# strukturag/libde265

Hardware: NVIDIA H100
Metric: decoded frames/sec at 4K Main profile, bit-exact YUV; MC kernel HBM GB/s (higher is better)
Workload: dtype u8

## Files before the change

libde265_b200/csrc/kernels_recon.cuh:

```cuda
#pragma once
#include "dev_common.cuh"
#include "kernels_residual.cuh"

#define RC_WARPS 8
#define RC_THREADS (RC_WARPS * 32)
#define RC_GSTRIDE 34
#define RC_TILE_STRIDE 40
#define RC_BLK (33 * RC_TILE_STRIDE + 8)
#define RC_FULL 0xffffffffu
#define RC_TRACE_WORDS 8

struct ReconArgs {
  const b200_tu* tus;
  const uint32_t* list;
  int n_list;
  int poll_ns;
  int region;
  int n_listw, n_list8;
  const uint32_t* task_start;
  int n_task;
  const b200_coeff* coeffs;
  const uint8_t* scaling;
  unsigned int* ticket;
  unsigned long long* trace;
  uint8_t* pend[3];
  int pend_w[3];
  const uint32_t* mark_list;
  int n_mark;
  unsigned int* err;
  unsigned int* err_host;
  unsigned long long spin_limit_ns;
};

struct ResidualSmem {
  int16_t coef[RC_WARPS][32 * RC_GSTRIDE];
  int16_t g[RC_WARPS][32 * RC_GSTRIDE];
  ResTables tb;
};

template <typename P>
struct IntraSmem {
  P blk[RC_WARPS][RC_BLK];
  int16_t coef[RC_WARPS][32 * RC_GSTRIDE];
  int16_t g[RC_WARPS][32 * RC_GSTRIDE];
  res_t res[RC_WARPS][32 * 32];
  P border[RC_WARPS][2][4 * 32 + 4];
  b200_tu tu_s[RC_WARPS][16];
  ResTables tb;
};

template <typename P, bool TO_RES>
__device__ void tu_residual(const b200_tu& tu, const b200_coeff* co, const uint8_t* __restrict__ scaling, P* dst, int dstride, res_t* res,
                            int bd, int16_t* coefT, int16_t* g, const ResTables& tb, int lane)
{
  const int log2 = tu.log2_size, nT = 1 << log2, n = tu.n_coeff;
  const int flags = tu.flags;
  const bool special = flags & (B200_TU_BYPASS | B200_TU_TSKIP);
  const Dequant dq = dequant_setup(tu, scaling, bd);
  int max_row = 0, max_col = 0;
  if (special) {
    max_row = max_col = nT - 1;
  } else {
    for (int i = lane; i < n; i += 32) {
      const int pos = co[i].pos;
      max_row = max(max_row, pos >> log2);
      max_col = max(max_col, pos & (nT - 1));
    }
    max_row = __reduce_max_sync(RC_FULL, max_row) & (nT - 1);
    max_col = __reduce_max_sync(RC_FULL, max_col) & (nT - 1);
  }
  const int nq = (max_row >> 2) + 1;
  uint32_t* cw = reinterpret_cast<uint32_t*>(coefT);
  uint32_t* gw = reinterpret_cast<uint32_t*>(g);
  constexpr int CW = RC_GSTRIDE / 2;
  for (int o = lane; o < (max_col + 1) * 2 * nq; o += 32) cw[(o / (2 * nq)) * CW + o % (2 * nq)] = 0;
  __syncwarp();
  for (int i = lane; i < n; i += 32) {
    const b200_coeff c = co[i];
    const int v = dequant_level(dq, c);
    const int pos = (dq.rotate ? (nT * nT - 1 - c.pos) : c.pos) & (nT * nT - 1);
    coefT[(pos & (nT - 1)) * RC_GSTRIDE + (pos >> log2)] = (int16_t)v;
  }
  __syncwarp();

  auto emit4 = [&](int x, int y, const int (&r)[4]) {
    if (TO_RES) res_store4(res + x + (y << log2), r[0], r[1], r[2], r[3]);
    else add_row<P, 4>(dst + x + (size_t)y * dstride, r, bd);
  };

  if (special) {
    const bool ts = !(flags & B200_TU_BYPASS);
    const int bd_shift = 20 - bd, ts_shift = 5 + log2, rnd = 1 << (bd_shift - 1);
    auto value = [&](int x, int y) {
      int c = coefT[x * RC_GSTRIDE + y];
      if (ts) c = ((int)((unsigned)c << ts_shift) + rnd) >> bd_shift;
      return c;
    };
    if (flags & (B200_TU_RDPCM_H | B200_TU_RDPCM_V)) {
      const bool vert = flags & B200_TU_RDPCM_V;
      if (lane < nT) {
        int sum = 0;
        for (int k = 0; k < nT; k++) {
          const int x = vert ? lane : k, y = vert ? k : lane;
          sum += value(x, y);
          if (TO_RES) res[x + (y << log2)] = (res_t)clip16(sum);
          else dst[x + (size_t)y * dstride] = (P)clip_bd((int)dst[x + (size_t)y * dstride] + sum, bd);
        }
      }
    } else {
      for (int o = lane; o < nT * nT / 4; o += 32) {
        const int x = (o & (nT / 4 - 1)) * 4, y = o >> (log2 - 2);
        const int r[4] = {value(x, y), value(x + 1, y), value(x + 2, y), value(x + 3, y)};
        emit4(x, y, r);
      }
    }
    __syncwarp();
    return;
  }

  const uint32_t* mt = (nT == 32) ? &tb.m32[0][0] : &tb.m16[0][0];
  const int post_shift = 20 - bd, rnd2 = 1 << (post_shift - 1);
  for (int o = lane; o < (max_col + 1) << (log2 - 2); o += 32) {
    const int ib = o & (nT / 4 - 1), c = o >> (log2 - 2);
    int acc[4] = {64, 64, 64, 64};
    const uint32_t* cp = cw + c * CW;
    for (int jq = 0; jq < nq; jq++) {
      const uint32_t c0 = cp[2 * jq], c1 = cp[2 * jq + 1];
      const uint4 m = *reinterpret_cast<const uint4*>(mt + jq * nT + 4 * ib);
      acc[0] = dp2a_hi(c1, m.x, dp2a_lo(c0, m.x, acc[0]));
      acc[1] = dp2a_hi(c1, m.y, dp2a_lo(c0, m.y, acc[1]));
      acc[2] = dp2a_hi(c1, m.z, dp2a_lo(c0, m.z, acc[2]));
      acc[3] = dp2a_hi(c1, m.w, dp2a_lo(c0, m.w, acc[3]));
    }
#pragma unroll
    for (int r = 0; r < 4; r++) g[(4 * ib + r) * RC_GSTRIDE + c] = (int16_t)clip16(acc[r] >> 7);
  }
  if ((max_col & 3) != 3) {
    const int c0 = max_col + 1, nc = 3 - (max_col & 3);
    for (int o = lane; o < nT * nc; o += 32) g[(o / nc) * RC_GSTRIDE + c0 + o % nc] = 0;
  }
  __syncwarp();
  const int nq2 = (max_col >> 2) + 1;
  for (int o = lane; o < nT << (log2 - 2); o += 32) {
    const int ib = o & (nT / 4 - 1), y = o >> (log2 - 2);
    int acc[4] = {rnd2, rnd2, rnd2, rnd2};
    const uint32_t* gp = gw + y * CW;
    for (int jq = 0; jq < nq2; jq++) {
      const uint32_t g0 = gp[2 * jq], g1 = gp[2 * jq + 1];
      const uint4 m = *reinterpret_cast<const uint4*>(mt + jq * nT + 4 * ib);
      acc[0] = dp2a_hi(g1, m.x, dp2a_lo(g0, m.x, acc[0]));
      acc[1] = dp2a_hi(g1, m.y, dp2a_lo(g0, m.y, acc[1]));
      acc[2] = dp2a_hi(g1, m.z, dp2a_lo(g0, m.z, acc[2]));
      acc[3] = dp2a_hi(g1, m.w, dp2a_lo(g0, m.w, acc[3]));
    }
    const int r[4] = {acc[0] >> post_shift, acc[1] >> post_shift, acc[2] >> post_shift, acc[3] >> post_shift};
    emit4(4 * ib, y, r);
  }
  __syncwarp();
}

__constant__ int8_t k_intra_angle[35] = {0,   0,   32,  26,  21,  17, 13, 9,  5,  2,  0,  -2, -5, -9, -13, -17, -21, -26,
                                         -32, -26, -21, -17, -13, -9, -5, -2, 0,  2,  5,  9,  13, 17, 21,  26,  32};
__constant__ int16_t k_inv_angle[15] = {-4096, -1638, -910, -630, -482, -390, -315, -256, -315, -390, -482, -630, -910, -1638, -4096};

template <typename P>
__device__ __forceinline__ void tu_intra_small(const b200_tu& tu, P* dst, int ts, int bd, bool filter_plane, const res_t* res, int lane)
{
  const int log2 = tu.log2_size, nT = 1 << log2, mode = tu.intra_mode, cidx = tu.cidx;
  const uint64_t avail = tu.avail;
  const int total = 4 * nT + 1;
  int v = 0, ve = 0;
  bool av = false, av_e = false;
  {
    const int i = lane - 2 * nT;
    if (lane < total) {
      if (i < 0) { const int r = -i - 1; av = (avail >> (r >> 2)) & 1; if (av) v = dst[-1 + r * ts]; }
      else if (i == 0) { av = (avail >> B200_AVAIL_CORNER_BIT) & 1; if (av) v = dst[-1 - ts]; }
      else { const int c = i - 1; av = (avail >> (B200_AVAIL_TOP_BIT0 + (c >> 2))) & 1; if (av) v = dst[c - ts]; }
    }
    if (nT == 8) {
      av_e = (avail >> (B200_AVAIL_TOP_BIT0 + 3)) & 1;
      if (av_e) ve = dst[15 - ts];
    }
  }
  {
    const unsigned m = __ballot_sync(RC_FULL, av);
    if (m == 0 && !av_e) {
      v = ve = 1 << (bd - 1);
    } else {
      const int first_lane = m ? __ffs(m) - 1 : 0;
      const int fv = __shfl_sync(RC_FULL, v, first_lane);
      const int first = m ? fv : ve;
      const unsigned below = m & ((2u << lane) - 1u);
      const int sv = __shfl_sync(RC_FULL, v, below ? 31 - __clz(below) : 0);
      v = below ? sv : first;
      const int last = __shfl_sync(RC_FULL, v, 31);
      if (!av_e) ve = last;
    }
  }
  if (filter_plane && nT == 8 && mode != 1) {
    const int d = min(abs(mode - 26), abs(mode - 10));
    if (d > 7) {
      const int vm = __shfl_up_sync(RC_FULL, v, 1);
      int vp = __shfl_down_sync(RC_FULL, v, 1);
      if (lane == 31) vp = ve;
      if (lane != 0) v = (vp + 2 * v + vm + 2) >> 2;
    }
  }
  auto B = [&](int i) -> int {
    const int s = i + 2 * nT;
    const int r = __shfl_sync(RC_FULL, v, s & 31);
    return (s == 32) ? ve : r;
  };
  const int npass = (nT == 4) ? 1 : 2;
  if (mode == 0) {
    const int tr = B(1 + nT), bl = B(-1 - nT);
    for (int p = 0; p < npass; p++) {
      const int o = lane + 32 * p, x = o & (nT - 1), y = (o >> log2) & (nT - 1);
      const int l = B(-1 - y), t = B(1 + x);
      int px = ((nT - 1 - x) * l + (x + 1) * tr + (nT - 1 - y) * t + (y + 1) * bl + nT) >> (log2 + 1);
      if (o < nT * nT) {
        if (res) px = clip_bd(px + res[o], bd);
        dst[x + y * ts] = (P)px;
      }
    }
  } else if (mode == 1) {
    const int i = lane - 2 * nT;
    const bool in = (i >= 1 && i <= nT) || (i <= -1 && i >= -nT);
    const int dc = (__reduce_add_sync(RC_FULL, in ? v : 0) + nT) >> (log2 + 1);
    const bool edge = (cidx == 0);
    const int b1 = B(1), bm1 = B(-1);
    for (int p = 0; p < npass; p++) {
      const int o = lane + 32 * p, x = o & (nT - 1), y = (o >> log2) & (nT - 1);
      const int t = B(x + 1), l = B(-y - 1);
      int px = dc;
      if (edge) {
        if (x == 0 && y == 0) px = (bm1 + 2 * dc + b1 + 2) >> 2;
        else if (y == 0) px = (t + 3 * dc + 2) >> 2;
        else if (x == 0) px = (l + 3 * dc + 2) >> 2;
      }
      if (o < nT * nT) {
        if (res) px = clip_bd(px + res[o], bd);
        dst[x + y * ts] = (P)px;
      }
    }
  } else {
    const int angle = k_intra_angle[mode];
    const bool vert = mode >= 18;
    const int sgn = vert ? 1 : -1;
    const int inv = (angle < 0) ? (int)k_inv_angle[mode - 11] : 0;
    const bool bfilt = (cidx == 0 && !(tu.flags & B200_TU_NO_BOUNDARY_FILTER) && (mode == 26 || mode == 10));
    const int b0 = B(0), b1 = B(1), bm1 = B(-1);
    auto R = [&](int k) -> int { return B(k >= 0 ? sgn * k : -sgn * ((k * inv + 128) >> 8)); };
    for (int p = 0; p < npass; p++) {
      const int o = lane + 32 * p, x = o & (nT - 1), y = (o >> log2) & (nT - 1);
      const int a = vert ? y : x, b = vert ? x : y;
      const int idx = ((a + 1) * angle) >> 5, fact = ((a + 1) * angle) & 31;
      const int r1 = R(b + idx + 1), r2 = R(b + idx + 2);
      const int l = B(-1 - y), t = B(1 + x);
      int px = fact ? ((32 - fact) * r1 + fact * r2 + 16) >> 5 : r1;
      if (bfilt) {
        if (mode == 26 && x == 0) px = clip_bd(b1 + ((l - b0) >> 1), bd);
        if (mode == 10 && y == 0) px = clip_bd(bm1 + ((t - b0) >> 1), bd);
      }
      if (o < nT * nT) {
        if (res) px = clip_bd(px + res[o], bd);
        dst[x + y * ts] = (P)px;
      }
    }
  }
  __syncwarp();
}

__device__ __forceinline__ bool intra_border_clamps(const b200_tu& tu, int& lo, int& hi)
{
  const int q = 1 << (tu.log2_size - 2);
  const uint64_t g = (1ull << q) - 1, av = tu.avail;
  if ((av & g) != g || !((av >> B200_AVAIL_CORNER_BIT) & 1) || ((av >> B200_AVAIL_TOP_BIT0) & g) != g) return false;
  const unsigned bl = (unsigned)((av >> q) & g), tr = (unsigned)((av >> (B200_AVAIL_TOP_BIT0 + q)) & g);
  if ((bl & (bl + 1)) || (tr & (tr + 1))) return false;
  lo = -4 * (q + __popc(bl));
  hi = 4 * (q + __popc(tr));
  return true;
}

struct TuDesc {
  uint32_t a, b;
  __device__ __forceinline__ int toff() const { return a & 1023; }
  __device__ __forceinline__ int mode() const { return (a >> 10) & 63; }
  __device__ __forceinline__ bool big() const { return (a >> 16) & 1; }
  __device__ __forceinline__ bool fast() const { return (a >> 17) & 1; }
  __device__ __forceinline__ bool smooth() const { return (a >> 18) & 1; }
  __device__ __forceinline__ bool bfilt() const { return (a >> 19) & 1; }
  __device__ __forceinline__ bool cbf() const { return (a >> 21) & 1; }
  __device__ __forceinline__ int rbase() const { return a >> 22; }
  __device__ __forceinline__ int plan_class() const { return (int)b; }
};

#define INTRA_PLAN_CLASSES (2 * 35 * 4 * 4 * 8)
__device__ uint32_t g_intra_plan[INTRA_PLAN_CLASSES][64];

inline void intra_plan_words(int cls, int lane, uint32_t (&w)[2])
{
  static const int8_t angle_of[35] = {0,   0,   32,  26,  21,  17, 13, 9,  5,  2,  0,  -2, -5, -9, -13, -17, -21, -26,
                                      -32, -26, -21, -17, -13, -9, -5, -2, 0,  2,  5,  9,  13, 17, 21,  26,  32};
  static const int16_t inv_of[15] = {-4096, -1638, -910, -630, -482, -390, -315, -256, -315, -390, -482, -630, -910, -1638, -4096};
  const bool smooth = cls & 1, bfilt = (cls >> 1) & 1, luma = (cls >> 2) & 1;
  const int hi2 = 4 * (((cls >> 3) & 3) + 1), lo2 = -4 * (((cls >> 5) & 3) + 1), mode = (cls >> 7) % 35, big = (cls >> 7) / 35;
  const int nT = big ? 8 : 4, log2 = big ? 3 : 2;
  auto O = [&](int i) -> uint32_t { i = std::min(std::max(i, lo2), hi2); return (uint32_t)(i < 0 ? -i * RC_TILE_STRIDE : i); };
  auto taps = [&](int i) -> uint32_t {
    if (smooth && i > -2 * nT && i < 2 * nT) return O(i - 1) | O(i) << 10 | O(i + 1) << 20;
    return O(i) * (1u | 1u << 10 | 1u << 20);
  };
  for (int p = 0; p < 2; p++) {
    const int o = lane + 32 * p, x = o & (nT - 1), y = (o >> log2) & (nT - 1);
    uint32_t v = 0;
    if (mode == 0) {
      if (p == 0 && lane <= 2 * nT + 2) v = taps(lane - nT - 1);
    } else if (mode == 1) {
      if (luma) {
        if (x == 0 && y == 0) v = O(-1) | O(1) << 10 | 2u << 20;
        else if (y == 0) v = O(x + 1) | 1u << 20;
        else if (x == 0) v = O(-y - 1) | 1u << 20;
      }
      const int i = lane - nT;
      if (p == 0 && lane < 2 * nT) v |= O(i < 0 ? i : i + 1) << 22;
    } else {
      const int angle = angle_of[mode], inv = angle < 0 ? inv_of[mode - 11] : 0, sgn = mode >= 18 ? 1 : -1;
      const int a = mode >= 18 ? y : x, b = mode >= 18 ? x : y;
      const int idx = ((a + 1) * angle) >> 5, fact = ((a + 1) * angle) & 31;
      auto R = [&](int k) -> int { return k >= 0 ? sgn * k : -sgn * ((k * inv + 128) >> 8); };
      if (smooth) v = taps(R(b + idx + 1));
      else v = O(R(b + idx + 1)) | O(R(b + idx + 2)) << 10 | (uint32_t)fact << 20;
      if (bfilt && mode == 26 && x == 0) v = O(1) | O(-1 - y) << 10 | 1u << 31;
      if (bfilt && mode == 10 && y == 0) v = O(-1) | O(1 + x) << 10 | 1u << 31;
    }
    w[p] = v;
  }
}

__device__ __forceinline__ TuDesc tu_desc(const b200_tu& tu, int G, bool filter_plane, int rbase)
{
  const int nT = 1 << tu.log2_size, mode = tu.intra_mode;
  int lo2 = 0, hi2 = 0;
  const bool fast = intra_border_clamps(tu, lo2, hi2);
  const bool smooth = nT == 8 && filter_plane && mode != 1 && min(abs(mode - 26), abs(mode - 10)) > 7;
  const bool bfilt = tu.cidx == 0 && !(tu.flags & B200_TU_NO_BOUNDARY_FILTER) && (mode == 26 || mode == 10);
  TuDesc d;
  d.a = (uint32_t)((tu.y & (G - 1)) * RC_TILE_STRIDE + (tu.x & (G - 1))) | (uint32_t)mode << 10 | (uint32_t)(nT == 8) << 16 | (uint32_t)fast << 17 |
        (uint32_t)smooth << 18 | (uint32_t)bfilt << 19 | (uint32_t)(tu.cidx == 0) << 20 | (uint32_t)((tu.flags & B200_TU_CBF) != 0) << 21 |
        (uint32_t)rbase << 22;
  d.b = fast ? (uint32_t)(((((nT == 8) * 35 + mode) * 4 + (-lo2 / 4 - 1)) * 4 + (hi2 / 4 - 1)) * 8 + (smooth | bfilt << 1 | (tu.cidx == 0) << 2)) : 0u;
  return d;
}

__device__ __forceinline__ TuDesc shfl_desc(const TuDesc& d, int src)
{
  return TuDesc{__shfl_sync(RC_FULL, d.a, src), __shfl_sync(RC_FULL, d.b, src)};
}

template <typename P, int LOG2>
__device__ __forceinline__ void tu_intra_fast(const TuDesc& d, P* dst, int ts, int bd, const int (&r)[2], const uint32_t (&w)[2], int lane)
{
  constexpr int nT = 1 << LOG2;
  constexpr int NP = (nT == 4) ? 1 : 2;
  const P* org = dst - ts - 1;
  auto T = [&](uint32_t u) -> int { return (int)org[u & 1023]; };
  auto F = [&](uint32_t u) -> int { return (T(u) + 2 * T(u >> 10) + T(u >> 20) + 2) >> 2; };
  const int mode = d.mode();
  int px[NP];
  if (mode == 0) {
    const int f = F(w[0]);
    const int tr = __shfl_sync(RC_FULL, f, 2 * nT + 2), bl = __shfl_sync(RC_FULL, f, 0);
#pragma unroll
    for (int p = 0; p < NP; p++) {
      const int o = lane + 32 * p, x = o & (nT - 1), y = (o >> LOG2) & (nT - 1);
      const int l = __shfl_sync(RC_FULL, f, nT - y), t = __shfl_sync(RC_FULL, f, nT + 2 + x);
      px[p] = ((nT - 1 - x) * l + (x + 1) * tr + (nT - 1 - y) * t + (y + 1) * bl + nT) >> (LOG2 + 1);
    }
  } else if (mode == 1) {
    const int dc = (__reduce_add_sync(RC_FULL, lane < 2 * nT ? T(w[0] >> 22) : 0) + nT) >> (LOG2 + 1);
#pragma unroll
    for (int p = 0; p < NP; p++) {
      const int kind = (w[p] >> 20) & 3, a = T(w[p]), b = kind == 2 ? T(w[p] >> 10) : dc;
      px[p] = kind ? (a + b + 2 * dc + 2) >> 2 : dc;
    }
  } else if (nT == 8 && d.smooth()) {
#pragma unroll
    for (int p = 0; p < NP; p++) px[p] = F(w[p]);
  } else {
#pragma unroll
    for (int p = 0; p < NP; p++) {
      const int r1 = T(w[p]), r2 = T(w[p] >> 10), fact = (w[p] >> 20) & 31;
      px[p] = ((32 - fact) * r1 + fact * r2 + 16) >> 5;
      if (d.bfilt() && (w[p] >> 31)) px[p] = clip_bd(r1 + ((r2 - (int)org[0]) >> 1), bd);
    }
  }
#pragma unroll
  for (int p = 0; p < NP; p++) {
    const int o = lane + 32 * p, x = o & (nT - 1), y = (o >> LOG2) & (nT - 1);
    if (o < nT * nT) dst[x + y * ts] = (P)clip_bd(px[p] + r[p], bd);
  }
  __syncwarp();
}

template <typename P>
__device__ void tu_intra_large(const b200_tu& tu, const P* gsrc, int gstride, P* dst, int bd, int bd_luma, uint32_t pic_flags, bool filter_plane,
                               P* b0mem, P* b1mem, int lane)
{
  const int log2 = tu.log2_size, nT = 1 << log2, mode = tu.intra_mode, cidx = tu.cidx, dstride = nT;
  const uint64_t avail = tu.avail;
  P* b0 = b0mem + 2 * 32 + 2;
  P* b1 = b1mem + 2 * 32 + 2;
  const int total = 4 * nT + 1;
  {
    constexpr int MAXC = 5;
    int v[MAXC];
    bool av[MAXC];
#pragma unroll
    for (int c5 = 0; c5 < MAXC; c5++) {
      const int s = 32 * c5 + lane, i = s - 2 * nT;
      av[c5] = false;
      v[c5] = 0;
      if (s < total) {
        const P* addr;
        if (i < 0) { const int r = -i - 1; av[c5] = (avail >> (r >> 2)) & 1; addr = gsrc - 1 + r * gstride; }
        else if (i == 0) { av[c5] = (avail >> B200_AVAIL_CORNER_BIT) & 1; addr = gsrc - 1 - gstride; }
        else { const int c = i - 1; av[c5] = (avail >> (B200_AVAIL_TOP_BIT0 + (c >> 2))) & 1; addr = gsrc + c - gstride; }
        if (av[c5]) v[c5] = (int)__ldcg(addr);
      }
    }
    int first_val = 1 << (bd - 1);
    bool any = false;
#pragma unroll
    for (int c5 = 0; c5 < MAXC; c5++) {
      const unsigned m = __ballot_sync(0xffffffffu, av[c5]);
      if (!any && m) { first_val = __shfl_sync(0xffffffffu, v[c5], __ffs(m) - 1); any = true; }
    }
    if (!any) {
      for (int s = lane; s < total; s += 32) b0[s - 2 * nT] = (P)(1 << (bd - 1));
    } else {
      int carry = first_val;
#pragma unroll
      for (int c5 = 0; c5 < MAXC; c5++) {
        if (32 * c5 < total) {
          const int s = 32 * c5 + lane, i = s - 2 * nT;
          const unsigned m = __ballot_sync(0xffffffffu, av[c5]);
          const unsigned below = m & ((2u << lane) - 1u);
          const int src = below ? 31 - __clz(below) : 0;
          const int sv = __shfl_sync(0xffffffffu, v[c5], src);
          const int outv = below ? sv : carry;
          if (s < total) b0[i] = (P)outv;
          carry = __shfl_sync(0xffffffffu, outv, 31);
        }
      }
    }
  }
  __syncwarp();
  const P* bsrc = b0;
  if (filter_plane && mode != 1) {
    const int d = min(abs(mode - 26), abs(mode - 10));
    const bool filt = d > ((nT == 8) ? 7 : (nT == 16) ? 1 : 0);
    if (filt) {
      const bool strong = (pic_flags & B200_PIC_STRONG_INTRA_SMOOTHING) && cidx == 0 && nT == 32 &&
                          abs((int)b0[0] + (int)b0[64] - 2 * (int)b0[32]) < (1 << (bd_luma - 5)) &&
                          abs((int)b0[0] + (int)b0[-64] - 2 * (int)b0[-32]) < (1 << (bd_luma - 5));
      for (int s = lane; s < total; s += 32) {
        const int i = s - 2 * nT;
        int v;
        if (i == -2 * nT || i == 2 * nT) v = b0[i];
        else if (strong) {
          if (i == 0) v = b0[0];
          else if (i < 0) v = (int)b0[0] + (((-i) * ((int)b0[-64] - (int)b0[0]) + 32) >> 6);
          else v = (int)b0[0] + ((i * ((int)b0[64] - (int)b0[0]) + 32) >> 6);
        } else v = ((int)b0[i + 1] + 2 * (int)b0[i] + (int)b0[i - 1] + 2) >> 2;
        b1[i] = (P)v;
      }
      __syncwarp();
      bsrc = b1;
    }
  }
  P* bfree = (bsrc == b0) ? b1 : b0;
  if (mode == 0) {
    for (int o = lane; o < nT * nT; o += 32) {
      const int x = o & (nT - 1), y = o >> log2;
      dst[x + y * dstride] = (P)(((nT - 1 - x) * (int)bsrc[-1 - y] + (x + 1) * (int)bsrc[1 + nT] + (nT - 1 - y) * (int)bsrc[1 + x] +
                                  (y + 1) * (int)bsrc[-1 - nT] + nT) >> (log2 + 1));
    }
  } else if (mode == 1) {
    int part = 0;
    for (int i = lane; i < nT; i += 32) part += (int)bsrc[i + 1] + (int)bsrc[-i - 1];
    const int dc = (__reduce_add_sync(RC_FULL, part) + nT) >> (log2 + 1);
    const bool edge = (cidx == 0 && nT < 32);
    for (int o = lane; o < nT * nT; o += 32) {
      const int x = o & (nT - 1), y = o >> log2;
      int v = dc;
      if (edge) {
        if (x == 0 && y == 0) v = ((int)bsrc[-1] + 2 * dc + (int)bsrc[1] + 2) >> 2;
        else if (y == 0) v = ((int)bsrc[x + 1] + 3 * dc + 2) >> 2;
        else if (x == 0) v = ((int)bsrc[-y - 1] + 3 * dc + 2) >> 2;
      }
      dst[x + y * dstride] = (P)v;
    }
  } else {
    const int angle = k_intra_angle[mode];
    const bool vert = mode >= 18;
    const int sgn = vert ? 1 : -1;
    P* ref = bfree;
    const int last = (nT * angle) >> 5;
    const int inv = (angle < 0) ? (int)k_inv_angle[mode - 11] : 0;
    const bool project = (angle < 0) && (last < -1);
    for (int s = lane; s <= 3 * nT; s += 32) {
      const int x = s - nT;
      const bool w = (x >= 0) ? (x <= nT || angle >= 0) : (project && x >= last);
      const int idx = (x >= 0) ? sgn * x : -sgn * ((x * inv + 128) >> 8);
      if (w) ref[x] = bsrc[idx];
    }
    __syncwarp();
    const bool bfilt = (cidx == 0 && nT < 32 && !(tu.flags & B200_TU_NO_BOUNDARY_FILTER) && (mode == 26 || mode == 10));
    for (int o = lane; o < nT * nT; o += 32) {
      const int x = o & (nT - 1), y = o >> log2;
      const int a = vert ? y : x, b = vert ? x : y;
      const int idx = ((a + 1) * angle) >> 5, fact = ((a + 1) * angle) & 31;
      int v = fact ? ((32 - fact) * (int)ref[b + idx + 1] + fact * (int)ref[b + idx + 2] + 16) >> 5 : (int)ref[b + idx + 1];
      if (bfilt) {
        if (mode == 26 && x == 0) v = clip_bd((int)bsrc[1] + (((int)bsrc[-1 - y] - (int)bsrc[0]) >> 1), bd);
        if (mode == 10 && y == 0) v = clip_bd((int)bsrc[-1] + (((int)bsrc[1 + x] - (int)bsrc[0]) >> 1), bd);
      }
      dst[x + y * dstride] = (P)v;
    }
  }
  __syncwarp();
}

template <typename P>
__device__ void tu_intra_large_clamped(const b200_tu& tu, int lo, int hi, P* gdst, int gstride, int bd, int bd_luma, uint32_t pic_flags,
                                       bool filter_plane, const res_t* res, P* bmem, int lane)
{
  const int log2 = tu.log2_size, nT = 1 << log2, mode = tu.intra_mode, cidx = tu.cidx;
  const int total = 4 * nT + 1;
  P* bs = bmem + 2 * 32 + 2;
  constexpr int MAXC = 5;
  int v[MAXC];
#pragma unroll
  for (int c5 = 0; c5 < MAXC; c5++) {
    const int s = 32 * c5 + lane, i = min(max(s - 2 * nT, lo), hi);
    v[c5] = 0;
    if (s < total) v[c5] = (int)__ldcg(i < 0 ? gdst - 1 + (-i - 1) * gstride : gdst + (i - 1) - gstride);
  }
  const bool filt = filter_plane && mode != 1 && min(abs(mode - 26), abs(mode - 10)) > ((nT == 16) ? 1 : 0);
  bool strong = false;
  int c0 = 0, bl = 0, tr = 0;
  if (filt && (pic_flags & B200_PIC_STRONG_INTRA_SMOOTHING) && cidx == 0 && nT == 32) {
    bl = __shfl_sync(RC_FULL, v[0], 0);
    const int ml = __shfl_sync(RC_FULL, v[1], 0);
    c0 = __shfl_sync(RC_FULL, v[2], 0);
    const int mt = __shfl_sync(RC_FULL, v[3], 0);
    tr = __shfl_sync(RC_FULL, v[4], 0);
    strong = abs(c0 + tr - 2 * mt) < (1 << (bd_luma - 5)) && abs(c0 + bl - 2 * ml) < (1 << (bd_luma - 5));
  }
#pragma unroll
  for (int c5 = 0; c5 < MAXC; c5++) {
    if (32 * c5 < total) {
      const int s = 32 * c5 + lane, i = s - 2 * nT;
      int f = v[c5];
      if (filt) {
        int vm = __shfl_up_sync(RC_FULL, v[c5], 1), vp = __shfl_down_sync(RC_FULL, v[c5], 1);
        const int vm_prev = (c5 > 0) ? __shfl_sync(RC_FULL, v[c5 > 0 ? c5 - 1 : 0], 31) : 0;
        const int vp_next = (c5 + 1 < MAXC) ? __shfl_sync(RC_FULL, v[c5 + 1 < MAXC ? c5 + 1 : c5], 0) : 0;
        if (lane == 0) vm = vm_prev;
        if (lane == 31) vp = vp_next;
        if (i == -2 * nT || i == 2 * nT) f = v[c5];
        else if (strong) f = (i == 0) ? c0 : (i < 0) ? c0 + (((-i) * (bl - c0) + 32) >> 6) : c0 + ((i * (tr - c0) + 32) >> 6);
        else f = (vp + 2 * v[c5] + vm + 2) >> 2;
      }
      if (s < total) bs[i] = (P)f;
    }
  }
  __syncwarp();
  auto emit = [&](int x, int y, int (&p)[4]) {
    if (res) {
      const uint2 rw = *reinterpret_cast<const uint2*>(res + x + (y << log2));
      p[0] += (int)(int16_t)(rw.x & 0xffff);
      p[1] += (int)(int16_t)(rw.x >> 16);
      p[2] += (int)(int16_t)(rw.y & 0xffff);
      p[3] += (int)(int16_t)(rw.y >> 16);
    }
#pragma unroll
    for (int k = 0; k < 4; k++) p[k] = clip_bd(p[k], bd);
    P* d = gdst + (size_t)y * gstride + x;
    if (sizeof(P) == 1) *reinterpret_cast<uint32_t*>(d) = (uint32_t)p[0] | (uint32_t)p[1] << 8 | (uint32_t)p[2] << 16 | (uint32_t)p[3] << 24;
    else *reinterpret_cast<uint2*>(d) = make_uint2((uint32_t)p[0] | (uint32_t)p[1] << 16, (uint32_t)p[2] | (uint32_t)p[3] << 16);
  };
  const int ngroups = nT * nT / 4;
  if (mode == 0) {
    const int trv = bs[1 + nT], blv = bs[-1 - nT];
    for (int g = lane; g < ngroups; g += 32) {
      const int x = (g & (nT / 4 - 1)) * 4, y = g >> (log2 - 2);
      const int l = bs[-1 - y];
      int p[4];
#pragma unroll
      for (int k = 0; k < 4; k++)
        p[k] = ((nT - 1 - x - k) * l + (x + k + 1) * trv + (nT - 1 - y) * (int)bs[1 + x + k] + (y + 1) * blv + nT) >> (log2 + 1);
      emit(x, y, p);
    }
  } else if (mode == 1) {
    const int part = (lane < nT) ? (int)bs[lane + 1] + (int)bs[-lane - 1] : 0;
    const int dc = (__reduce_add_sync(RC_FULL, part) + nT) >> (log2 + 1);
    const bool edge = (cidx == 0 && nT < 32);
    for (int g = lane; g < ngroups; g += 32) {
      const int x = (g & (nT / 4 - 1)) * 4, y = g >> (log2 - 2);
      int p[4];
#pragma unroll
      for (int k = 0; k < 4; k++) {
        int vv = dc;
        if (edge) {
          if (x + k == 0 && y == 0) vv = ((int)bs[-1] + 2 * dc + (int)bs[1] + 2) >> 2;
          else if (y == 0) vv = ((int)bs[x + k + 1] + 3 * dc + 2) >> 2;
          else if (x + k == 0) vv = ((int)bs[-y - 1] + 3 * dc + 2) >> 2;
        }
        p[k] = vv;
      }
      emit(x, y, p);
    }
  } else {
    const int angle = k_intra_angle[mode];
    const bool vert = mode >= 18;
    const int sgn = vert ? 1 : -1;
    const int inv = (angle < 0) ? (int)k_inv_angle[mode - 11] : 0;
    const bool bfilt = (cidx == 0 && nT < 32 && !(tu.flags & B200_TU_NO_BOUNDARY_FILTER) && (mode == 26 || mode == 10));
    auto R = [&](int k) -> int { return bs[k >= 0 ? sgn * min(k, 2 * nT) : -sgn * ((k * inv + 128) >> 8)]; };
    for (int g = lane; g < ngroups; g += 32) {
      const int x = (g & (nT / 4 - 1)) * 4, y = g >> (log2 - 2);
      int p[4];
#pragma unroll
      for (int k = 0; k < 4; k++) {
        const int a = vert ? y : x + k, b = vert ? x + k : y;
        const int idx = ((a + 1) * angle) >> 5, fact = ((a + 1) * angle) & 31;
        const int r1 = R(b + idx + 1), r2 = R(b + idx + 2);
        int vv = ((32 - fact) * r1 + fact * r2 + 16) >> 5;
        if (bfilt) {
          if (mode == 26 && x + k == 0) vv = clip_bd((int)bs[1] + (((int)bs[-1 - y] - (int)bs[0]) >> 1), bd);
          if (mode == 10 && y == 0) vv = clip_bd((int)bs[-1] + (((int)bs[1 + x + k] - (int)bs[0]) >> 1), bd);
        }
        p[k] = vv;
      }
      emit(x, y, p);
    }
  }
}

template <typename P>
__device__ __forceinline__ void block_store(const P* blk, uint8_t* plane, int pitch, int x, int y, int nT, int lane)
{
  const int upr = nT * (int)sizeof(P) / 4;
  for (int o = lane; o < nT * upr; o += 32) {
    const int r = o / upr, u = o % upr;
    *reinterpret_cast<uint32_t*>(plane + (size_t)(y + r) * pitch + (size_t)x * sizeof(P) + 4 * u) = reinterpret_cast<const uint32_t*>(blk + r * nT)[u];
  }
}

template <typename P>
__global__ void __launch_bounds__(RC_THREADS) k_residual(DevPic pic, ReconArgs args)
{
  __shared__ ResidualSmem sm;
  const int tid = threadIdx.x, warp = tid >> 5, lane = tid & 31;
  for (int i = tid; i < (int)(sizeof(ResTables) / 4); i += RC_THREADS) reinterpret_cast<uint32_t*>(&sm.tb)[i] = reinterpret_cast<const uint32_t*>(&c_res)[i];
  for (int i = blockIdx.x * RC_THREADS + tid; i < args.n_mark; i += gridDim.x * RC_THREADS) {
    const b200_tu tu = args.tus[args.mark_list[i]];
    const int c = tu.cidx, n4u = 1 << (tu.log2_size - 2);
    uint8_t* p = args.pend[c] + (tu.y >> 2) * args.pend_w[c] + (tu.x >> 2);
    for (int j = 0; j < n4u; j++)
      for (int k = 0; k < n4u; k++) p[j * args.pend_w[c] + k] = 1;
  }
  __syncthreads();
  const int n4 = args.n_list - args.n_listw - args.n_list8;
  const int Ww = args.n_listw, W8 = (args.n_list8 + 3) >> 2, W4 = (n4 + 31) >> 5;
  uint32_t* scratch = reinterpret_cast<uint32_t*>(sm.coef[warp]);
  for (int wi = blockIdx.x * RC_WARPS + warp; wi < Ww + W8 + W4; wi += gridDim.x * RC_WARPS) {
    if (wi < Ww) {
      const b200_tu tu = args.tus[args.list[wi]];
      const int c = tu.cidx, nT = 1 << tu.log2_size;
      P* dst = row_ptr<P>(pic.cur[c], pic.pitch[c], tu.y) + tu.x;
      const int dstride = pic.pitch[c] / (int)sizeof(P);
      if (tu.flags & B200_TU_PCM) {
        for (int i = lane; i < tu.n_coeff; i += 32) {
          const b200_coeff co = args.coeffs[tu.coeff_off + i];
          dst[(co.pos & (nT - 1)) + (co.pos >> tu.log2_size) * dstride] = (P)(uint16_t)co.level;
        }
      } else {
        tu_residual<P, false>(tu, args.coeffs + tu.coeff_off, args.scaling, dst, dstride, nullptr, c ? pic.bd_c : pic.bd_y, sm.coef[warp], sm.g[warp],
                              sm.tb, lane);
      }
    } else if (wi < Ww + W8) {
      const int idx = Ww + (wi - Ww) * 4 + (lane >> 3);
      const bool active = idx < Ww + args.n_list8;
      b200_tu tu;
      if (active) tu = args.tus[args.list[idx]];
      else { tu.x = tu.y = 0; tu.cidx = 0; tu.coeff_off = 0; }
      const int c = tu.cidx;
      P* dst = row_ptr<P>(pic.cur[c], pic.pitch[c], tu.y) + tu.x;
      res8_quarter<P, false>(active, tu, args.coeffs + tu.coeff_off, args.scaling, dst, pic.pitch[c] / (int)sizeof(P), nullptr, c ? pic.bd_c : pic.bd_y,
                             scratch + (lane >> 3) * 64, lane & 7, sm.tb);
    } else {
      const int idx = Ww + args.n_list8 + (wi - Ww - W8) * 32 + lane;
      if (idx < args.n_list) {
        const b200_tu tu = args.tus[args.list[idx]];
        const int c = tu.cidx;
        P* dst = row_ptr<P>(pic.cur[c], pic.pitch[c], tu.y) + tu.x;
        res4_lane<P, false>(tu, args.coeffs + tu.coeff_off, args.scaling, dst, pic.pitch[c] / (int)sizeof(P), nullptr, c ? pic.bd_c : pic.bd_y, scratch, lane,
                            sm.tb);
      }
    }
    __syncwarp();
  }
}

__global__ void k_mark_pending(ReconArgs args)
{
  const int idx = blockIdx.x * blockDim.x + threadIdx.x;
  if (idx >= args.n_list) return;
  const b200_tu tu = args.tus[args.list[idx]];
  const int c = tu.cidx, n4 = 1 << (tu.log2_size - 2);
  uint8_t* p = args.pend[c] + (tu.y >> 2) * args.pend_w[c] + (tu.x >> 2);
  for (int j = 0; j < n4; j++)
    for (int i = 0; i < n4; i++) p[j * args.pend_w[c] + i] = 1;
}

__device__ __forceinline__ void dep_units_of(const b200_tu& tu, int rx, int ry, int span, unsigned& left, bool& corner, unsigned& top)
{
  const int half = 1 << (tu.log2_size - 1);
  const int ux0 = (tu.x - rx) >> 2, uy0 = (tu.y - ry) >> 2;
  const uint64_t avail = tu.avail;
  const unsigned gm = (half >= 32) ? 0xffffffffu : ((1u << half) - 1u), sm = (1u << span) - 1u;
  const bool cb = (avail >> B200_AVAIL_CORNER_BIT) & 1;
  if (ux0 == 0) {
    left |= (((unsigned)avail & gm) << uy0) & sm;
    if (cb) { if (uy0 == 0) corner = true; else left |= 1u << (uy0 - 1); }
  } else if (uy0 == 0 && cb) {
    top |= 1u << (ux0 - 1);
  }
  if (uy0 == 0) top |= (((unsigned)(avail >> B200_AVAIL_TOP_BIT0) & gm) << ux0) & sm;
}

__device__ __forceinline__ unsigned ld_acquire_u8(const uint8_t* p)
{
  unsigned v;
  asm volatile("ld.acquire.gpu.global.u8 %0, [%1];" : "=r"(v) : "l"(p) : "memory");
  return v;
}
__device__ __forceinline__ void st_relaxed_u8(uint8_t* p, unsigned v) { asm volatile("st.relaxed.gpu.global.u8 [%0], %1;" ::"l"(p), "r"(v) : "memory"); }

template <typename P>
__global__ void __launch_bounds__(RC_THREADS, 3) k_intra(DevPic pic, ReconArgs args)
{
  extern __shared__ __align__(16) uint8_t smem_raw[];
  IntraSmem<P>& sm = *reinterpret_cast<IntraSmem<P>*>(smem_raw);
  const int tid = threadIdx.x, warp = tid >> 5, lane = tid & 31;
  for (int i = tid; i < (int)(sizeof(ResTables) / 4); i += RC_THREADS) reinterpret_cast<uint32_t*>(&sm.tb)[i] = reinterpret_cast<const uint32_t*>(&c_res)[i];
  __syncthreads();
  b200_tu* tus = sm.tu_s[warp];
  res_t* res = sm.res[warp];
  P* blk = sm.blk[warp];
  for (;;) {
    unsigned t = 0;
    if (lane == 0) t = atomicAdd(args.ticket, 1u);
    t = __shfl_sync(RC_FULL, t, 0);
    if (t >= (unsigned)args.n_task) return;
    unsigned tr_c = 0;
    auto tr_time = [&](int w) {
      if (args.trace && lane == 0) {
        unsigned long long g;
        asm volatile("mov.u64 %0, %%globaltimer;" : "=l"(g));
        args.trace[(unsigned long long)RC_TRACE_WORDS * t + w] = g;
      }
    };
    auto tr_cycles = [&](int w) {
      if (args.trace && lane == 0) {
        const unsigned c = (unsigned)clock();
        if (w >= 0) args.trace[(unsigned long long)RC_TRACE_WORDS * t + w] += c - tr_c;
        tr_c = c;
      }
    };
    tr_time(0);
    tr_cycles(-1);
    const uint32_t first = args.task_start[t], count = min(args.task_start[t + 1] - first, 16u);
    if (lane < (int)count) tus[lane] = args.tus[args.list[first + lane]];
    __syncwarp();
    const b200_tu tu0 = tus[0];
    const int G0 = args.region >> (tu0.cidx ? 1 : 0);
    const bool region = (1 << tu0.log2_size) <= min(G0, 8);
    unsigned seg_starts;
    {
      const int mc = (lane < (int)count) ? tus[lane].cidx : -1, pc = (lane > 0 && lane < (int)count) ? tus[lane - 1].cidx : -1;
      seg_starts = __ballot_sync(RC_FULL, lane < (int)count && (lane == 0 || mc != pc));
    }
    TuDesc desc{0u, 0u};
    {
      const bool mine = lane < (int)count;
      const b200_tu& mytu = tus[mine ? lane : 0];
      const int l2 = mytu.log2_size, sz = mine ? 1 << (2 * l2) : 0;
      const int mybd = mytu.cidx ? pic.bd_c : pic.bd_y;
      int incl = sz;
#pragma unroll
      for (int d = 1; d < 16; d <<= 1) {
        const int up = __shfl_up_sync(RC_FULL, incl, d);
        if (lane >= d) incl += up;
      }
      const int my_rbase = incl - sz;
      if (region && mine) {
        const int c = mytu.cidx;
        desc = tu_desc(mytu, args.region >> (c ? 1 : 0), !(pic.flags & B200_PIC_INTRA_SMOOTHING_OFF) && (c == 0 || pic.chroma == 3), my_rbase);
      }
      const bool cbf = mine && (mytu.flags & B200_TU_CBF);
      const unsigned m8 = __ballot_sync(RC_FULL, cbf && l2 == 3), mw = __ballot_sync(RC_FULL, cbf && l2 > 3);
      uint32_t* scratch = reinterpret_cast<uint32_t*>(sm.coef[warp]);
      if (cbf && l2 == 2) res4_lane<P, true>(mytu, args.coeffs + mytu.coeff_off, args.scaling, nullptr, 0, res + my_rbase, mybd, scratch, lane, sm.tb);
      __syncwarp();
      for (unsigned rem = m8; rem;) {
        const int q = lane >> 3;
        const unsigned idx = __fns(rem, 0, q + 1);
        const bool active = idx < 32u;
        const b200_tu& tu = tus[active ? idx : 0];
        const int rb = __shfl_sync(RC_FULL, my_rbase, active ? idx : 0);
        res8_quarter<P, true>(active, tu, args.coeffs + tu.coeff_off, args.scaling, nullptr, 0, res + rb, tu.cidx ? pic.bd_c : pic.bd_y, scratch + q * 64,
                              lane & 7, sm.tb);
#pragma unroll
        for (int k = 0; k < 4; k++) rem &= rem - 1;
      }
      for (unsigned rem = mw; rem; rem &= rem - 1) {
        const int idx = __ffs(rem) - 1;
        const b200_tu& tu = tus[idx];
        const int rb = __shfl_sync(RC_FULL, my_rbase, idx);
        tu_residual<P, true>(tu, args.coeffs + tu.coeff_off, args.scaling, nullptr, 0, res + rb, tu.cidx ? pic.bd_c : pic.bd_y, sm.coef[warp], sm.g[warp],
                             sm.tb, lane);
      }
    }
    uint32_t w[2] = {0u, 0u};
    if (region) {
      const int cls = shfl_desc(desc, 0).plan_class();
      w[0] = __ldg(&g_intra_plan[cls][lane]);
      w[1] = __ldg(&g_intra_plan[cls][lane + 32]);
    }
    tr_cycles(3);
    for (unsigned ss = seg_starts; ss; ss &= ss - 1) {
      const int s0 = __ffs(ss) - 1, s1 = (ss & (ss - 1)) ? __ffs(ss & (ss - 1)) - 1 : (int)count;
      const b200_tu& ts0 = tus[s0];
      const int c = ts0.cidx, G = args.region >> (c ? 1 : 0);
      const int rx = region ? ts0.x & ~(G - 1) : ts0.x, ry = region ? ts0.y & ~(G - 1) : ts0.y;
      const int span = region ? (2 * G) >> 2 : (1 << ts0.log2_size) >> 1;
      unsigned left = 0, top = 0;
      bool corner = false;
      if (lane >= s0 && lane < s1) dep_units_of(tus[lane], rx, ry, span, left, corner, top);
      left = __reduce_or_sync(RC_FULL, left);
      top = __reduce_or_sync(RC_FULL, top);
      corner = __any_sync(RC_FULL, corner);
      const int pw = args.pend_w[c];
      const uint8_t* pend = args.pend[c] + (ry >> 2) * pw + (rx >> 2);
      const uint8_t* f = nullptr;
      if (lane < span) { if ((left >> lane) & 1) f = pend + lane * pw - 1; }
      else if (lane == span) { if (corner) f = pend - pw - 1; }
      else if (lane - span - 1 < span) { if ((top >> (lane - span - 1)) & 1) f = pend - pw + (lane - span - 1); }
      const uint8_t* f2 = nullptr;
      if (span == 16 && lane == 0 && ((top >> 15) & 1)) f2 = pend - pw + 15;
      unsigned ns = 32, spins = 0;
      unsigned long long t_wait0 = 0;
      for (;;) {
        const bool busy = (f && ld_acquire_u8(f)) || (f2 && ld_acquire_u8(f2));
        if (!__any_sync(RC_FULL, busy)) break;
        __nanosleep(ns);
        if (ns < (unsigned)args.poll_ns) ns *= 2;
        else if ((++spins & 63u) == 0) {
          unsigned long long now;
          asm volatile("mov.u64 %0, %%globaltimer;" : "=l"(now));
          if (!t_wait0) t_wait0 = now;
          bool give_up = now - t_wait0 > args.spin_limit_ns || *(volatile unsigned int*)args.err != 0;
          give_up = __shfl_sync(RC_FULL, give_up, 0);
          if (give_up) {
            if (lane == 0) {
              atomicCAS(args.err, 0u, t + 1);
              *(volatile unsigned int*)args.err_host = t + 1;
              __threadfence_system();
            }
            break;
          }
        }
      }
    }
    __syncwarp();
    tr_time(1);
    tr_cycles(4);

    if (!region) {
      const int c = tu0.cidx, bd = c ? pic.bd_c : pic.bd_y;
      const bool filter_plane = !(pic.flags & B200_PIC_INTRA_SMOOTHING_OFF) && (c == 0 || pic.chroma == 3);
      const int nT = 1 << tu0.log2_size;
      const int gstride = pic.pitch[c] / (int)sizeof(P);
      P* gdst = row_ptr<P>(pic.cur[c], pic.pitch[c], tu0.y) + tu0.x;
      int lo = 0, hi = 0;
      if (nT >= 16 && intra_border_clamps(tu0, lo, hi)) {
        tu_intra_large_clamped<P>(tu0, lo, hi, gdst, gstride, bd, pic.bd_y, pic.flags, filter_plane, (tu0.flags & B200_TU_CBF) ? res : nullptr,
                                  sm.border[warp][0], lane);
        tr_cycles(6);
      } else {
        tu_intra_large<P>(tu0, gdst, gstride, blk, bd, pic.bd_y, pic.flags, filter_plane, sm.border[warp][0], sm.border[warp][1], lane);
        if (tu0.flags & B200_TU_CBF) {
          for (int o = lane; o < nT * nT; o += 32) blk[o] = (P)clip_bd((int)blk[o] + res[o], bd);
          __syncwarp();
        }
        tr_cycles(6);
        block_store<P>(blk, pic.cur[c], pic.pitch[c], tu0.x, tu0.y, nT, lane);
      }
    } else {
      for (unsigned ss = seg_starts; ss; ss &= ss - 1) {
        const int s0 = __ffs(ss) - 1, s1 = (ss & (ss - 1)) ? __ffs(ss & (ss - 1)) - 1 : (int)count;
        const b200_tu& ts0 = tus[s0];
        const int c = ts0.cidx, bd = c ? pic.bd_c : pic.bd_y, G = args.region >> (c ? 1 : 0);
        const int rx = ts0.x & ~(G - 1), ry = ts0.y & ~(G - 1);
        const bool filter_plane = !(pic.flags & B200_PIC_INTRA_SMOOTHING_OFF) && (c == 0 || pic.chroma == 3);
        const int pwid = c ? pic.cw : pic.w, phei = c ? pic.ch : pic.h;
        int covered = 0;
        for (int i = s0; i < s1; i++) covered += 1 << (2 * tus[i].log2_size);
        const int TS = RC_TILE_STRIDE;
        P* tile = blk + TS + 4;
        const int gw = min(G, pwid - rx), gh = min(G, phei - ry);
        const bool full = (gw == G) && (gh == G);
        tr_cycles(-1);
        const bool interior = covered < gw * gh;
        constexpr int NW = 2 * (int)sizeof(P);
        const int wpr = G * (int)sizeof(P) / 4;
        uint32_t in_w[NW];
        if (interior && full) {
#pragma unroll
          for (int k = 0; k < NW; k++) {
            const int o = lane + 32 * k;
            if (o < G * wpr) in_w[k] = __ldcg(reinterpret_cast<const uint32_t*>(row_ptr<P>(pic.cur[c], pic.pitch[c], ry + o / wpr) + rx) + o % wpr);
          }
        }
        const int xt0 = lane - 1, xt1 = lane + 31;
        const bool top0 = ry > 0 && xt0 < 2 * G && rx + xt0 >= 0 && rx + xt0 < pwid;
        const bool top1 = ry > 0 && xt1 < 2 * G && rx + xt1 < pwid;
        const bool left = rx > 0 && lane < 2 * G && ry + lane < phei;
        P top_s0, top_s1, left_s;
        if (top0) top_s0 = __ldcg(row_ptr<P>(pic.cur[c], pic.pitch[c], ry - 1) + rx + xt0);
        if (top1) top_s1 = __ldcg(row_ptr<P>(pic.cur[c], pic.pitch[c], ry - 1) + rx + xt1);
        if (left) left_s = __ldcg(row_ptr<P>(pic.cur[c], pic.pitch[c], ry + lane) + rx - 1);
        if (interior && full) {
#pragma unroll
          for (int k = 0; k < NW; k++) {
            const int o = lane + 32 * k;
            if (o < G * wpr) reinterpret_cast<uint32_t*>(tile + (o / wpr) * TS)[o % wpr] = in_w[k];
          }
        } else if (interior) {
          for (int o = lane; o < gw * gh; o += 32) {
            const int x = o % gw, y = o / gw;
            tile[y * TS + x] = __ldcg(row_ptr<P>(pic.cur[c], pic.pitch[c], ry + y) + rx + x);
          }
        }
        if (top0) tile[-TS + xt0] = top_s0;
        if (top1) tile[-TS + xt1] = top_s1;
        if (left) tile[lane * TS - 1] = left_s;
        __syncwarp();
        tr_cycles(5);
        TuDesc d = shfl_desc(desc, s0);
        for (int i = s0; i < s1; i++) {
          const TuDesc dn = shfl_desc(desc, (i + 1) & 31);
          const uint32_t wn[2] = {__ldg(&g_intra_plan[dn.plan_class()][lane]), __ldg(&g_intra_plan[dn.plan_class()][lane + 32])};
          P* tdst = tile + d.toff();
          const res_t* tres = d.cbf() ? res + d.rbase() : nullptr;
          if (!d.fast()) {
            tu_intra_small<P>(tus[i], tdst, TS, bd, filter_plane, tres, lane);
          } else {
            const int n = d.big() ? 64 : 16;
            int r[2] = {0, 0};
            if (tres) {
              if (lane < n) r[0] = tres[lane];
              if (lane + 32 < n) r[1] = tres[lane + 32];
            }
            if (d.big()) tu_intra_fast<P, 3>(d, tdst, TS, bd, r, w, lane);
            else tu_intra_fast<P, 2>(d, tdst, TS, bd, r, w, lane);
          }
          d = dn;
          w[0] = wn[0];
          w[1] = wn[1];
        }
        tr_cycles(6);
        if (full) {
          const int wpr = G * (int)sizeof(P) / 4;
          for (int o = lane; o < G * wpr; o += 32) {
            const int y = o / wpr, u = o % wpr;
            reinterpret_cast<uint32_t*>(row_ptr<P>(pic.cur[c], pic.pitch[c], ry + y) + rx)[u] = reinterpret_cast<const uint32_t*>(tile + y * TS)[u];
          }
        } else {
          for (int o = lane; o < gw * gh; o += 32) {
            const int x = o % gw, y = o / gw;
            row_ptr<P>(pic.cur[c], pic.pitch[c], ry + y)[rx + x] = tile[y * TS + x];
          }
        }
        __syncwarp();
      }
    }
    __syncwarp();
    if (lane < (int)count) {
      asm volatile("fence.release.gpu;" ::: "memory");
      const b200_tu& tu = tus[lane];
      const int n4 = 1 << (tu.log2_size - 2), pw = args.pend_w[tu.cidx];
      uint8_t* pend = args.pend[tu.cidx] + (tu.y >> 2) * pw + (tu.x >> 2);
      for (int j = 0; j < n4; j++)
        for (int i = 0; i < n4; i++) st_relaxed_u8(pend + j * pw + i, 0);
    }
    __syncwarp();
    tr_time(2);
    if (args.trace && lane == 0)
      args.trace[(unsigned long long)RC_TRACE_WORDS * t + 7] = count | ((unsigned long long)tu0.cidx << 8) | ((unsigned long long)tu0.log2_size << 16);
  }
}
```

Before: 3305.

## Stage per-task intra plan words into shared memory with cp.async prefetch

Each TU's intra plan table entries are now copied from global memory into a per-warp shared buffer with cp.async at task start, packed by a warp prefix sum over per-TU word counts (16 for 4x4, 64 for 8x8). The copy overlaps the residual and dependency wait. The per-TU __ldg prefetch of plan words in the intra loop is replaced by shared-memory reads at a stored offset. TUs that overflow the 384-word budget fall back to the slow path, and the sm.g buffer is reused, which risks conflicts with the residual code's use of it.

```diff
diff --git a/libde265_b200/csrc/kernels_recon.cuh b/libde265_b200/csrc/kernels_recon.cuh
--- a/libde265_b200/csrc/kernels_recon.cuh
+++ b/libde265_b200/csrc/kernels_recon.cuh
@@ -294,11 +294,15 @@
   __device__ __forceinline__ bool bfilt() const { return (a >> 19) & 1; }
   __device__ __forceinline__ bool cbf() const { return (a >> 21) & 1; }
   __device__ __forceinline__ int rbase() const { return a >> 22; }
-  __device__ __forceinline__ int plan_class() const { return (int)b; }
+  __device__ __forceinline__ int plan_class() const { return (int)(b & 0xffff); }
+  __device__ __forceinline__ int plan_off() const { return (int)(b >> 16); }
 };
 
 #define INTRA_PLAN_CLASSES (2 * 35 * 4 * 4 * 8)
-__device__ uint32_t g_intra_plan[INTRA_PLAN_CLASSES][64];
+__device__ __align__(16) uint32_t g_intra_plan[INTRA_PLAN_CLASSES][64];
+
+__host__ __device__ __forceinline__ int intra_plan_nwords(int cls) { return cls >= INTRA_PLAN_CLASSES / 2 ? 64 : 16; }
+#define RC_PLAN_WORDS 384
 
 inline void intra_plan_words(int cls, int lane, uint32_t (&w)[2])
 {
@@ -316,6 +320,10 @@
   for (int p = 0; p < 2; p++) {
     const int o = lane + 32 * p, x = o & (nT - 1), y = (o >> log2) & (nT - 1);
     uint32_t v = 0;
+    if (o >= intra_plan_nwords(cls)) {
+      w[p] = 0;
+      continue;
+    }
     if (mode == 0) {
       if (p == 0 && lane <= 2 * nT + 2) v = taps(lane - nT - 1);
     } else if (mode == 1) {
@@ -361,10 +369,13 @@
 }
 
 template <typename P, int LOG2>
-__device__ __forceinline__ void tu_intra_fast(const TuDesc& d, P* dst, int ts, int bd, const int (&r)[2], const uint32_t (&w)[2], int lane)
+__device__ __forceinline__ void tu_intra_fast(const TuDesc& d, P* dst, int ts, int bd, const int (&r)[2], const uint32_t* plan, int lane)
 {
   constexpr int nT = 1 << LOG2;
   constexpr int NP = (nT == 4) ? 1 : 2;
+  uint32_t w[NP];
+  w[0] = (nT == 8 || lane < 16) ? plan[lane] : 0u;
+  if (NP == 2) w[NP - 1] = plan[lane + 32];
   const P* org = dst - ts - 1;
   auto T = [&](uint32_t u) -> int { return (int)org[u & 1023]; };
   auto F = [&](uint32_t u) -> int { return (T(u) + 2 * T(u >> 10) + T(u >> 20) + 2) >> 2; };
@@ -797,6 +808,10 @@
       seg_starts = __ballot_sync(RC_FULL, lane < (int)count && (lane == 0 || mc != pc));
     }
     TuDesc desc{0u, 0u};
+    static_assert(RC_PLAN_WORDS % 128 == 0 && RC_PLAN_WORDS / 16 <= 32 && RC_PLAN_WORDS * 4 <= sizeof(sm.g[0]) &&
+                      offsetof(IntraSmem<P>, g) % 16 == 0 && sizeof(sm.g[0]) % 16 == 0,
+                  "the staged plan words fit a warp's 16-byte aligned g buffer, one chunk bit per 16 words");
+    uint32_t* plan_s = reinterpret_cast<uint32_t*>(sm.g[warp]);
     {
       const bool mine = lane < (int)count;
       const b200_tu& mytu = tus[mine ? lane : 0];
@@ -812,6 +827,35 @@
       if (region && mine) {
         const int c = mytu.cidx;
         desc = tu_desc(mytu, args.region >> (c ? 1 : 0), !(pic.flags & B200_PIC_INTRA_SMOOTHING_OFF) && (c == 0 || pic.chroma == 3), my_rbase);
+      }
+      if (region) {
+        int nw = desc.fast() ? intra_plan_nwords(desc.plan_class()) : 0;
+        int wincl = nw;
+#pragma unroll
+        for (int d = 1; d < 16; d <<= 1) {
+          const int up = __shfl_up_sync(RC_FULL, wincl, d);
+          if (lane >= d) wincl += up;
+        }
+        if (wincl > RC_PLAN_WORDS) {
+          desc.a &= ~(1u << 17);
+          nw = 0;
+        }
+        const int off = wincl - nw;
+        desc.b |= (uint32_t)off << 16;
+        const unsigned owners = __ballot_sync(RC_FULL, nw != 0);
+        const unsigned starts = __reduce_or_sync(RC_FULL, nw ? 1u << (off >> 4) : 0u);
+        const int nchunk = __reduce_max_sync(RC_FULL, nw ? (off + nw) >> 4 : 0);
+        const unsigned upto = starts & ((2u << lane) - 1u);
+        const int owner = __fns(owners, 0, max(__popc(upto), 1));
+        const int src_cls = TuDesc{0u, __shfl_sync(RC_FULL, desc.b, owner < 32 ? owner : 0)}.plan_class();
+        const int src = src_cls * 16 + (lane - (upto ? 31 - __clz(upto) : 0)) * 4;
+        const uint4* table = reinterpret_cast<const uint4*>(&g_intra_plan[0][0]);
+        const unsigned dst0 = (unsigned)__cvta_generic_to_shared(plan_s);
+#pragma unroll
+        for (int k = 0; k < RC_PLAN_WORDS / 128; k++) {
+          const int q = lane + 32 * k, sq = __shfl_sync(RC_FULL, src, (q >> 2) & 31);
+          if ((q >> 2) < nchunk) asm volatile("cp.async.cg.shared.global [%0], [%1], 16;" ::"r"(dst0 + 16 * q), "l"(table + sq + (q & 3)) : "memory");
+        }
       }
       const bool cbf = mine && (mytu.flags & B200_TU_CBF);
       const unsigned m8 = __ballot_sync(RC_FULL, cbf && l2 == 3), mw = __ballot_sync(RC_FULL, cbf && l2 > 3);
@@ -836,12 +880,6 @@
         tu_residual<P, true>(tu, args.coeffs + tu.coeff_off, args.scaling, nullptr, 0, res + rb, tu.cidx ? pic.bd_c : pic.bd_y, sm.coef[warp], sm.g[warp],
                              sm.tb, lane);
       }
-    }
-    uint32_t w[2] = {0u, 0u};
-    if (region) {
-      const int cls = shfl_desc(desc, 0).plan_class();
-      w[0] = __ldg(&g_intra_plan[cls][lane]);
-      w[1] = __ldg(&g_intra_plan[cls][lane + 32]);
     }
     tr_cycles(3);
     for (unsigned ss = seg_starts; ss; ss &= ss - 1) {
@@ -888,6 +926,7 @@
         }
       }
     }
+    asm volatile("cp.async.wait_all;" ::: "memory");
     __syncwarp();
     tr_time(1);
     tr_cycles(4);
@@ -966,7 +1005,6 @@
         TuDesc d = shfl_desc(desc, s0);
         for (int i = s0; i < s1; i++) {
           const TuDesc dn = shfl_desc(desc, (i + 1) & 31);
-          const uint32_t wn[2] = {__ldg(&g_intra_plan[dn.plan_class()][lane]), __ldg(&g_intra_plan[dn.plan_class()][lane + 32])};
           P* tdst = tile + d.toff();
           const res_t* tres = d.cbf() ? res + d.rbase() : nullptr;
           if (!d.fast()) {
@@ -978,12 +1016,10 @@
               if (lane < n) r[0] = tres[lane];
               if (lane + 32 < n) r[1] = tres[lane + 32];
             }
-            if (d.big()) tu_intra_fast<P, 3>(d, tdst, TS, bd, r, w, lane);
-            else tu_intra_fast<P, 2>(d, tdst, TS, bd, r, w, lane);
+            if (d.big()) tu_intra_fast<P, 3>(d, tdst, TS, bd, r, plan_s + d.plan_off(), lane);
+            else tu_intra_fast<P, 2>(d, tdst, TS, bd, r, plan_s + d.plan_off(), lane);
           }
           d = dn;
-          w[0] = wn[0];
-          w[1] = wn[1];
         }
         tr_cycles(6);
         if (full) {
```

Result: no change. 3288, median of 6 (-0.5%).
